# rakhimovv/lvt

Measured on AMD Instinct MI355X. Metric: video-clips/sec/node (VQVAE+DSFVT train step, BAIR 64x64x16), higher is better.
Workload: dtype f32

## Files before the change

### lvt_amd/csrc/attention_flash.hip

```cpp
#include "attn_common.h"

namespace {

template <int I> struct IC { static constexpr int value = I; };
template <int N, int I = 0, class F> __device__ __forceinline__ void static_for(F &&f) {
    if constexpr (I < N) { f(IC<I>{}); static_for<N, I + 1>(f); }
}

typedef _Float16 f16x8 __attribute__((ext_vector_type(8)));
typedef _Float16 f16x2v __attribute__((ext_vector_type(2)));
typedef float f32x2 __attribute__((ext_vector_type(2)));
typedef float f32x4v __attribute__((ext_vector_type(4)));
typedef short s16x4 __attribute__((ext_vector_type(4)));
typedef __attribute__((address_space(3))) s16x4 lds_s16x4;
typedef unsigned u32x4 __attribute__((ext_vector_type(4)));

#define FA_LD 144
#define FA_PL (64 * FA_LD)
#define FA_SLOT (2 * FA_PL)
#define FA_EMIN 30
#define FA_EMAX 254
#define FA_LOG2E 1.4426950408889634f

typedef unsigned u32x2 __attribute__((ext_vector_type(2)));
// ... 13 lines not shown
    v = fa_dpp_max<0x140>(v);
    return v;
}
__device__ __forceinline__ float fa_kg_max(float v) {
    u32x2 r = __builtin_amdgcn_permlane16_swap(__float_as_uint(v), __float_as_uint(v), false, false);
    v = fmaxf(fa_u2f(r[0]), fa_u2f(r[1]));
    r = __builtin_amdgcn_permlane32_swap(__float_as_uint(v), __float_as_uint(v), false, false);
    return fmaxf(fa_u2f(r[0]), fa_u2f(r[1]));
}
__device__ __forceinline__ float fa_kg_sum(float v) {
    u32x2 r = __builtin_amdgcn_permlane16_swap(__float_as_uint(v), __float_as_uint(v), false, false);
    v = fa_u2f(r[0]) + fa_u2f(r[1]);
    r = __builtin_amdgcn_permlane32_swap(__float_as_uint(v), __float_as_uint(v), false, false);
    return fa_u2f(r[0]) + fa_u2f(r[1]);
}
__device__ __forceinline__ float fa_max4(const f32x4v a) { return fmaxf(fmaxf(a[0], a[1]), fmaxf(a[2], a[3])); }
__device__ __forceinline__ float fa_absmax4(const float4 a) { return fmaxf(fmaxf(fabsf(a.x), fabsf(a.y)), fmaxf(fabsf(a.z), fabsf(a.w))); }

__device__ __forceinline__ float fa_mix_lo(unsigned h, float c) {
    float r;
    asm("v_fma_mix_f32 %0, %1, %2, %3 op_sel:[0,0,0] op_sel_hi:[1,0,0]" : "=v"(r) : "v"(h), "v"(-1.f), "v"(c));
    return r;
}
__device__ __forceinline__ float fa_mix_hi(unsigned h, float c) {
    float r;
    asm("v_fma_mix_f32 %0, %1, %2, %3 op_sel:[1,0,0] op_sel_hi:[1,0,0]" : "=v"(r) : "v"(h), "v"(-1.f), "v"(c));
    return r;
}
__device__ __forceinline__ void fa_split_pair(float a, float b, float s, unsigned &ph, unsigned &pl) {
    const f32x2 t = f32x2{a, b} * s;
    ph = __builtin_bit_cast(unsigned, __builtin_convertvector(t, f16x2v));
    const f32x2 r = {fa_mix_lo(ph, t.x), fa_mix_hi(ph, t.y)};
    pl = __builtin_bit_cast(unsigned, __builtin_convertvector(r, f16x2v));
}
__device__ __forceinline__ void fa_split_pair1(float a, float b, unsigned &ph, unsigned &pl) {
    const f32x2 t = {a, b};
    ph = __builtin_bit_cast(unsigned, __builtin_convertvector(t, f16x2v));
    const f32x2 r = {fa_mix_lo(ph, a), fa_mix_hi(ph, b)};
    pl = __builtin_bit_cast(unsigned, __builtin_convertvector(r, f16x2v));
}
__device__ __forceinline__ void fa_split8(const float (&v)[8], f16x8 &h, f16x8 &l) {
    u32x4 uh, ul;
    unsigned a, b;
    fa_split_pair1(v[0], v[1], a, b); uh[0] = a; ul[0] = b;
    fa_split_pair1(v[2], v[3], a, b); uh[1] = a; ul[1] = b;
    fa_split_pair1(v[4], v[5], a, b); uh[2] = a; ul[2] = b;
    fa_split_pair1(v[6], v[7], a, b); uh[3] = a; ul[3] = b;
    h = __builtin_bit_cast(f16x8, uh);
    l = __builtin_bit_cast(f16x8, ul);
}
__device__ __forceinline__ float fa_score(float acc, float kq, float bias) { return fmaf(acc, kq, bias); }
__device__ __forceinline__ f32x4v fa_mfma(const f16x8 a, const f16x8 b, const f32x4v c) {
    return __builtin_amdgcn_mfma_f32_16x16x32_f16(a, b, c, 0, 0, 0);
}

__device__ __forceinline__ int fa_row_scale(const float4 a, const float4 b) {
    return fa_ebits(fa_row16_max(fmaxf(fa_absmax4(a), fa_absmax4(b))));
}
__device__ __forceinline__ void fa_row_store(const float4 a, const float4 b, int eb, unsigned short *slot, float *rs_inv, int row, int c) {
    const float s = fa_u2f((unsigned)(268 - eb) << 23);
    uint2 h0, l0, h1, l1;
    fa_split_pair(a.x, a.y, s, h0.x, l0.x); fa_split_pair(a.z, a.w, s, h0.y, l0.y);
    fa_split_pair(b.x, b.y, s, h1.x, l1.x); fa_split_pair(b.z, b.w, s, h1.y, l1.y);
    unsigned short *d = slot + row * FA_LD + 4 * c;
    *reinterpret_cast<uint2 *>(d) = h0;
    *reinterpret_cast<uint2 *>(d + 64) = h1;
    *reinterpret_cast<uint2 *>(d + FA_PL) = l0;
    *reinterpret_cast<uint2 *>(d + FA_PL + 64) = l1;
    rs_inv[c == 0 ? row : 64 + c] = fa_u2f((unsigned)(eb - 14) << 23);
}
struct G4 { float4 v[4]; };
__device__ __forceinline__ void fa_load(G4 &g, const float *__restrict__ x, const float *__restrict__ y, long long ld, int tid) {
    const int r = tid >> 4, c = tid & 15;
    const float *px = x + (long long)r * ld + 4 * c, *py = y + (long long)r * ld + 4 * c;
    g.v[0] = *reinterpret_cast<const float4 *>(px);
    g.v[1] = *reinterpret_cast<const float4 *>(px + 64);
    g.v[2] = *reinterpret_cast<const float4 *>(py);
    g.v[3] = *reinterpret_cast<const float4 *>(py + 64);
}
__device__ __forceinline__ void fa_park(const G4 &g, unsigned short *slot, float *rs_inv, int tid) {
    const int r = tid >> 4, c = tid & 15;
#pragma unroll
    for (int half = 0; half < 2; ++half)
        fa_row_store(g.v[2 * half], g.v[2 * half + 1], fa_row_scale(g.v[2 * half], g.v[2 * half + 1]), slot, rs_inv, 32 * half + r, c);
}
struct G8 { float4 v[8]; };
__device__ __forceinline__ void fa_load8(G8 &g, const float *__restrict__ x, const float *__restrict__ y, long long ld, int tid) {
    const int r = tid >> 4, c = tid & 15;
    const float *px = x + (long long)r * ld + 4 * c, *py = y + (long long)r * ld + 4 * c;
    g.v[0] = *reinterpret_cast<const float4 *>(px);
    g.v[1] = *reinterpret_cast<const float4 *>(px + 64);
    g.v[2] = *reinterpret_cast<const float4 *>(px + 16 * ld);
    g.v[3] = *reinterpret_cast<const float4 *>(px + 16 * ld + 64);
    g.v[4] = *reinterpret_cast<const float4 *>(py);
    g.v[5] = *reinterpret_cast<const float4 *>(py + 64);
    g.v[6] = *reinterpret_cast<const float4 *>(py + 16 * ld);
    g.v[7] = *reinterpret_cast<const float4 *>(py + 16 * ld + 64);
}
__device__ __forceinline__ void fa_park8(const G8 &g, unsigned short *slot, float *rs_inv, int tid) {
    const int r = tid >> 4, c = tid & 15;
#pragma unroll
    for (int p = 0; p < 4; ++p)
        fa_row_store(g.v[2 * p], g.v[2 * p + 1], fa_row_scale(g.v[2 * p], g.v[2 * p + 1]), slot, rs_inv, 16 * p + r, c);
}
__device__ __forceinline__ void fa_bfrags_request(const float *__restrict__ row, int kg, float4 (&v)[8]) {
#pragma unroll
    for (int s = 0; s < 4; ++s) {
        v[2 * s] = *reinterpret_cast<const float4 *>(row + 32 * s + 8 * kg);
        v[2 * s + 1] = *reinterpret_cast<const float4 *>(row + 32 * s + 8 * kg + 4);
    }
}
__device__ __forceinline__ void fa_bfrags_split(const float4 (&v)[8], f16x8 (&fr)[4][2], float &inv) {
    float m = 0.f;
#pragma unroll
    for (int e = 0; e < 8; ++e) m = fmaxf(m, fa_absmax4(v[e]));
    m = fa_kg_max(m);
    const int eb = fa_ebits(m);
    const float sc = fa_u2f((unsigned)(268 - eb) << 23);
    inv = fa_u2f((unsigned)(eb - 14) << 23);
#pragma unroll
    for (int s = 0; s < 4; ++s) {
        u32x4 uh, ul;
        unsigned a, b;
        fa_split_pair(v[2 * s].x, v[2 * s].y, sc, a, b); uh[0] = a; ul[0] = b;
        fa_split_pair(v[2 * s].z, v[2 * s].w, sc, a, b); uh[1] = a; ul[1] = b;
        fa_split_pair(v[2 * s + 1].x, v[2 * s + 1].y, sc, a, b); uh[2] = a; ul[2] = b;
        fa_split_pair(v[2 * s + 1].z, v[2 * s + 1].w, sc, a, b); uh[3] = a; ul[3] = b;
        fr[s][0] = __builtin_bit_cast(f16x8, uh);
        fr[s][1] = __builtin_bit_cast(f16x8, ul);
    }
}
__device__ __forceinline__ void fa_load_bfrags(const float *__restrict__ row, int kg, f16x8 (&fr)[4][2], float &inv) {
    float4 v[8];
    fa_bfrags_request(row, kg, v);
    fa_bfrags_split(v, fr, inv);
}
__device__ __forceinline__ f16x8 fa_rowfrag(const unsigned short *slot, int pl, int row, int s, int kg) {
    return *reinterpret_cast<const f16x8 *>(slot + pl * FA_PL + row * FA_LD + 32 * s + 8 * kg);
}
__device__ __forceinline__ f16x8 fa_trfrag(const unsigned short *slot, int pl, int rb, int dtile, int c16, int kg) {
    const unsigned short *p = slot + pl * FA_PL + (rb + 4 * kg + (c16 >> 2)) * FA_LD + 16 * dtile + 4 * (c16 & 3);
    const s16x4 lo = __builtin_amdgcn_ds_read_tr16_b64_v4i16((lds_s16x4 *)(p));
    const s16x4 hi = __builtin_amdgcn_ds_read_tr16_b64_v4i16((lds_s16x4 *)(p + 16 * FA_LD));
    union { struct { s16x4 a, b; } s; f16x8 v; } u;
    u.s.a = lo; u.s.b = hi;
    return u.v;
}

struct FaSmem {
    unsigned short ring[2][FA_SLOT];
    float rs_inv[2][80];
    float dhs[32];
};
template <int NR> struct FaSmemA {
    unsigned short ring[2][FA_SLOT];
    float rs_inv[2][80];
    float dhs[32];
    float red[16];
    float R[128 * 4 * NR];
};
struct FaSmem3 {
    unsigned short ring[3][FA_SLOT];
    float rs_inv[3][80];
    float dhs[32];
};

__device__ __forceinline__ int fa_pair(unsigned x) { return (int)(((x >> 4) << 3) | (x & 7)); }
__device__ __forceinline__ int fa_half(unsigned x) { return (int)((x >> 3) & 1); }
__device__ __forceinline__ int fa_pair4(unsigned x) { return (int)(((x >> 5) << 3) | (x & 7)); }
__device__ __forceinline__ int fa_quarter(unsigned x) { return (int)((x >> 3) & 3); }
__device__ __forceinline__ int fa_opaque(int x) { asm volatile("" : "+s"(x)); return x; }

template <int BH, int BW> struct Geo16 {
    static_assert(BW == 16 || BW == 8, "16-wide tiles: BW is 8 or 16");
    static constexpr int HP = BW == 16 ? BH : BH / 2;
    static __device__ __forceinline__ int hj(int hslot, int kg) { return BW == 16 ? hslot : 2 * hslot + (kg >> 1); }
    static __device__ __forceinline__ int wj(int r, int kg) { return BW == 16 ? 4 * kg + r : 4 * (kg & 1) + r; }
};
template <int BT, int BH, int BW> struct BankIdx {
    static constexpr int NT = 2 * BT - 1, NH = 2 * BH - 1, NW = 2 * BW - 1, NB = NT + NH + NW;
};

struct FaArgs {
    const float *q, *k, *v, *d_o;
    long long ld;
    int H;
    float c1, fill2;
    float inv_temper;
    const float *dt, *dh, *dw;
    float *o, *m, *l;
    float *dq, *dk, *dv, *delta, *scal, *bank_partial;
};

template <int BT, int BH, int BW, int MASKED, int NCH>
__device__ __forceinline__ float fa_fwd_body(const FaArgs &A, FaSmem &sm, int bh_, int qhalf) {
    using GE = Geo16<BH, BW>;
    constexpr int HP = GE::HP;
    static_assert(BT * BH * BW == AT_S, "256 tokens");
    const int tid = threadIdx.x, lane = tid & 63, wave = tid >> 6;
    const int c16 = lane & 15, kg = lane >> 4;
    const int b = bh_ / A.H, h = bh_ % A.H;
    const long long row0 = (long long)b * AT_S;
    const int il = wave * 16 + c16, i = qhalf * 128 + il;
    const float *kbase = A.k + row0 * A.ld + h * AT_D, *vbase = A.v + row0 * A.ld + h * AT_D;
    constexpr int NIT = NCH;

    if (tid < 2 * BH - 1) sm.dhs[tid] = A.dh[h * (2 * BH - 1) + tid] * FA_LOG2E;
    G4 g0, g1;
#define FA_G(t) ((((t) & 1) == 0) ? g0 : g1)
    auto load_item = [&](int t, G4 &gg) { fa_load(gg, kbase + (long long)(32 * t) * A.ld, vbase + (long long)(32 * t) * A.ld, A.ld, tid); };
    load_item(0, g0);
    if (NIT > 1) load_item(1, g1);
    f16x8 qb[4][2];
    float qinv;
    fa_load_bfrags(A.q + (row0 + i) * A.ld + h * AT_D, kg, qb, qinv);
    const int wi = i % BW, hi = (i / BW) % BH, ti = i / (BW * BH);
    float bt_[BT], bw_[4];
#pragma unroll
    for (int x = 0; x < BT; ++x) bt_[x] = A.dt[h * (2 * BT - 1) + ti - x + BT - 1] * FA_LOG2E;
#pragma unroll
    for (int r = 0; r < 4; ++r) bw_[r] = A.dw[h * (2 * BW - 1) + wi - GE::wj(r, kg) + BW - 1] * FA_LOG2E;
    const float *dhl = sm.dhs + (hi + BH - 1 - (BW == 16 ? 0 : (kg >> 1)));
    constexpr int HSTEP = BW == 16 ? 1 : 2;
    const float qc = qinv * A.c1;
    fa_park(g0, sm.ring[0], sm.rs_inv[0], tid);
    __syncthreads();

    f32x4v oacc[AT_D / 16];
#pragma unroll
    for (int d = 0; d < AT_D / 16; ++d) oacc[d] = f32x4v{0.f, 0.f, 0.f, 0.f};
    float m_run = -3.0e38f, lsum = 0.f;
    float vmax_run = fa_u2f((unsigned)(FA_EMIN - 14) << 23);

    static_for<NIT>([&](auto tc) {
        constexpr int t = decltype(tc)::value;
        const unsigned short *cur = sm.ring[t & 1];
        const float *cinv = sm.rs_inv[t & 1];
        if constexpr (t + 2 < NIT) load_item(t + 2, FA_G(t));
        f32x4v st[2] = {f32x4v{0.f, 0.f, 0.f, 0.f}, f32x4v{0.f, 0.f, 0.f, 0.f}};
#pragma unroll
        for (int s = 0; s < 4; ++s) {
            f16x8 a[2][2];
#pragma unroll
            for (int kt = 0; kt < 2; ++kt)
#pragma unroll
                for (int pl = 0; pl < 2; ++pl) a[kt][pl] = fa_rowfrag(cur, pl, 16 * kt + c16, s, kg);
#pragma unroll
            for (int kt = 0; kt < 2; ++kt) st[kt] = fa_mfma(a[kt][1], qb[s][0], st[kt]);
#pragma unroll
            for (int kt = 0; kt < 2; ++kt) st[kt] = fa_mfma(a[kt][0], qb[s][1], st[kt]);
#pragma unroll
            for (int kt = 0; kt < 2; ++kt) st[kt] = fa_mfma(a[kt][0], qb[s][0], st[kt]);
        }
        if constexpr (t + 1 < NIT) fa_park(FA_G(t + 1), sm.ring[(t + 1) & 1], sm.rs_inv[(t + 1) & 1], tid);
        float x[8];
        f32x4v vinv[2];
#pragma unroll
        for (int kt = 0; kt < 2; ++kt) {
            const int T = 2 * t + kt;
            const f32x4v kinv = *reinterpret_cast<const f32x4v *>(cinv + 16 * kt + 4 * kg);
            vinv[kt] = *reinterpret_cast<const f32x4v *>(cinv + 32 + 16 * kt + 4 * kg);
            const float bth = bt_[T / HP] + dhl[-HSTEP * (T % HP)];
#pragma unroll
            for (int r = 0; r < 4; ++r) {
                float v = fa_score(st[kt][r], kinv[r] * qc, bth + bw_[r]);
                if (MASKED && 16 * T + 4 * kg + r > i) v = A.fill2;
                x[4 * kt + r] = v;
            }
        }
        float cmax = fmaxf(fmaxf(fmaxf(x[0], x[1]), fmaxf(x[2], x[3])), fmaxf(fmaxf(x[4], x[5]), fmaxf(x[6], x[7])));
        cmax = fa_kg_max(cmax);
        const float vmax_c = fa_kg_max(fmaxf(fa_max4(vinv[0]), fa_max4(vinv[1])));
        const float m_new = fmaxf(m_run, cmax);
        const float alpha = __builtin_amdgcn_exp2f(m_run - m_new);
        m_run = m_new;
        const float vmax_new = fmaxf(vmax_run, vmax_c);
        const float fo = alpha * (vmax_run * __builtin_amdgcn_rcpf(vmax_new));
        vmax_run = vmax_new;
        const float srun = 32768.f * __builtin_amdgcn_rcpf(vmax_new);
        float psum = 0.f, pw[8];
#pragma unroll
        for (int kt = 0; kt < 2; ++kt)
#pragma unroll
            for (int r = 0; r < 4; ++r) {
                const float p = __builtin_amdgcn_exp2f(x[4 * kt + r] - m_new);
                psum += p;
                pw[4 * kt + r] = p * (vinv[kt][r] * srun);
            }
        lsum = lsum * alpha + psum;
        f16x8 pbh, pbl;
        fa_split8(pw, pbh, pbl);
#pragma unroll
        for (int d = 0; d < AT_D / 16; ++d) oacc[d] *= fo;
#pragma unroll
        for (int dp = 0; dp < AT_D / 32; ++dp) {
            f16x8 a[2][2];
#pragma unroll
            for (int dd = 0; dd < 2; ++dd)
#pragma unroll
                for (int pl = 0; pl < 2; ++pl) a[dd][pl] = fa_trfrag(cur, pl, 32, 2 * dp + dd, c16, kg);
#pragma unroll
            for (int dd = 0; dd < 2; ++dd) oacc[2 * dp + dd] = fa_mfma(a[dd][1], pbh, oacc[2 * dp + dd]);
#pragma unroll
            for (int dd = 0; dd < 2; ++dd) oacc[2 * dp + dd] = fa_mfma(a[dd][0], pbl, oacc[2 * dp + dd]);
#pragma unroll
            for (int dd = 0; dd < 2; ++dd) oacc[2 * dp + dd] = fa_mfma(a[dd][0], pbh, oacc[2 * dp + dd]);
        }
        __syncthreads();
    });
#undef FA_G
    const float linv = 1.f / fa_kg_sum(lsum);
    const float osc = (vmax_run * (1.f / 32768.f)) * linv;
    float am = 0.f;
    {
        float *orow = A.o + (row0 + i) * A.ld + h * AT_D + 4 * kg;
#pragma unroll
        for (int d = 0; d < AT_D / 16; ++d) {
            const f32x4v ov = oacc[d] * osc;
            *reinterpret_cast<f32x4v *>(orow + 16 * d) = ov;
            am = fmaxf(am, fmaxf(fmaxf(fabsf(ov[0]), fabsf(ov[1])), fmaxf(fabsf(ov[2]), fabsf(ov[3]))));
        }
    }
    if (kg == 0) {
        const long long si = ((long long)b * A.H + h) * AT_S + i;
        A.m[si] = m_run;
        A.l[si] = linv;
    }
    return am;
}

template <int BT, int BH, int BW, int MASKED>
__global__ __launch_bounds__(512, 1) void lvt_attn_fwd_flash_kernel(const FaArgs A, float *__restrict__ o_amax) {
    __shared__ __attribute__((aligned(16))) FaSmem sm;
    if (threadIdx.x >= 256) __builtin_amdgcn_s_setprio(1);
    float am;
    if (MASKED) {
        am = fa_fwd_body<BT, BH, BW, MASKED, 8>(A, sm, blockIdx.x, 1);
        __syncthreads();
        am = fmaxf(am, fa_fwd_body<BT, BH, BW, MASKED, 4>(A, sm, fa_opaque(blockIdx.x), 0));
    } else {
        am = fa_fwd_body<BT, BH, BW, MASKED, 8>(A, sm, fa_pair(blockIdx.x), fa_half(blockIdx.x));
    }
    if (o_amax) {
        __syncthreads();
        lvt_block_amax_commit(am, o_amax, reinterpret_cast<float *>(sm.ring[0]));
    }
}

template <int BT, int BH, int BW, int MASKED, int NCH, int ONEP>
__device__ __forceinline__ float fa_bwd_a_body(const FaArgs &A, FaSmemA<BT + Geo16<BH, BW>::HP + 4> &sm, int bh_, int qhalf) {
    using GE = Geo16<BH, BW>;
    using BI = BankIdx<BT, BH, BW>;
    constexpr int HP = GE::HP;
    constexpr int NR = BT + HP + 4;
    static_assert(BT * BH * BW == AT_S, "256 tokens");
    const int tid = threadIdx.x, lane = tid & 63, wave = tid >> 6;
    const int c16 = lane & 15, kg = lane >> 4;
    const int b = bh_ / A.H, h = bh_ % A.H;
    const long long row0 = (long long)b * AT_S;
    const int il = wave * 16 + c16, i = qhalf * 128 + il;
    const float *kbase = A.k + row0 * A.ld + h * AT_D, *vbase = A.v + row0 * A.ld + h * AT_D;
    constexpr int NIT = ONEP ? NCH : 2 * NCH;

    if (tid < 2 * BH - 1) sm.dhs[tid] = A.dh[h * (2 * BH - 1) + tid] * FA_LOG2E;
    float *mine = sm.R + (il * 4 + kg) * NR;
#pragma unroll
    for (int x = 0; x < NR; ++x) mine[x] = 0.f;
    G4 g0;
    auto load_item = [&](int t, G4 &gg) {
        const int c = t < NCH ? t : t - NCH;
        fa_load(gg, kbase + (long long)(32 * c) * A.ld, vbase + (long long)(32 * c) * A.ld, A.ld, tid);
    };
    load_item(0, g0);
    f16x8 qb[4][2], dob[4][2];
    float qinv, doinv;
    float4 qraw[8], doraw[8], oraw[ONEP ? 8 : 1];
    fa_bfrags_request(A.q + (row0 + i) * A.ld + h * AT_D, kg, qraw);
    fa_bfrags_request(A.d_o + (row0 + i) * A.ld + h * AT_D, kg, doraw);
    if constexpr (ONEP) fa_bfrags_request(A.o + (row0 + i) * A.ld + h * AT_D, kg, oraw);
    fa_bfrags_split(qraw, qb, qinv);
    fa_bfrags_split(doraw, dob, doinv);
    float delta_early = 0.f;
    if constexpr (ONEP) {
        float a0 = 0.f, a1 = 0.f;
#pragma unroll
        for (int s_ = 0; s_ < 4; ++s_) {
            const float4 o0 = oraw[2 * s_], o1 = oraw[2 * s_ + 1], d0 = doraw[2 * s_], d1 = doraw[2 * s_ + 1];
            a0 = fmaf(o0.x, d0.x, a0); a0 = fmaf(o0.y, d0.y, a0); a0 = fmaf(o0.z, d0.z, a0); a0 = fmaf(o0.w, d0.w, a0);
            a1 = fmaf(o1.x, d1.x, a1); a1 = fmaf(o1.y, d1.y, a1); a1 = fmaf(o1.z, d1.z, a1); a1 = fmaf(o1.w, d1.w, a1);
        }
        delta_early = fa_kg_sum(a0 + a1);
    }
    const long long si = ((long long)b * A.H + h) * AT_S + i;
    const float m_i = A.m[si], linv = A.l[si];
    const int wi = i % BW, hi = (i / BW) % BH, ti = i / (BW * BH);
    float bt_[BT];
    f32x4v bw4;
#pragma unroll
    for (int x = 0; x < BT; ++x) bt_[x] = A.dt[h * (2 * BT - 1) + ti - x + BT - 1] * FA_LOG2E;
#pragma unroll
    for (int r = 0; r < 4; ++r) bw4[r] = A.dw[h * (2 * BW - 1) + wi - GE::wj(r, kg) + BW - 1] * FA_LOG2E;
    const float *dhl = sm.dhs + (hi + BH - 1 - (BW == 16 ? 0 : (kg >> 1)));
    constexpr int HSTEP = BW == 16 ? 1 : 2;
    const float qc = qinv * A.c1;
    fa_park(g0, sm.ring[0], sm.rs_inv[0], tid);
    load_item(1, g0);
    __syncthreads();

    float delta = 0.f, gmax = 0.f;
    float kmax = fa_u2f((unsigned)(FA_EMIN - 14) << 23);
    float sgf = 0.f, kmr = 0.f, dl = 0.f;
    int ebG = FA_EMIN;
    if constexpr (ONEP) { delta = delta_early; dl = delta * linv; }
    f32x4v qacc[AT_D / 16];
#pragma unroll
    for (int d = 0; d < AT_D / 16; ++d) qacc[d] = f32x4v{0.f, 0.f, 0.f, 0.f};
    constexpr bool CORR = ONEP;
    f32x4v cacc[CORR ? AT_D / 16 : 1];
#pragma unroll
    for (int d = 0; d < (CORR ? AT_D / 16 : 1); ++d) cacc[d] = f32x4v{0.f, 0.f, 0.f, 0.f};
    int ebC = 16;
    float rst[BT], rsw[4];
#pragma unroll
    for (int x = 0; x < BT; ++x) rst[x] = 0.f;
#pragma unroll
    for (int r = 0; r < 4; ++r) rsw[r] = 0.f;

    static_for<NIT>([&](auto tc) {
        constexpr int t = decltype(tc)::value;
        constexpr int c = t < NCH ? t : t - NCH;
        constexpr bool PASS2 = ONEP || t >= NCH;
        const unsigned short *cur = sm.ring[t & 1];
        const float *cinv = sm.rs_inv[t & 1];
        constexpr bool PARK = t + 1 < NIT;
        unsigned short *nslot = sm.ring[(t + 1) & 1];
        float *ninv = sm.rs_inv[(t + 1) & 1];
        if constexpr (!ONEP && t == NCH) {
            delta = fa_kg_sum(delta) * linv;
            gmax = fa_kg_max(gmax);
            kmax = fa_kg_max(kmax);
            const float G = gmax + fabsf(delta);
            ebG = fa_ebits(G);
            sgf = fa_u2f((unsigned)(268 - ebG) << 23);
            kmr = __builtin_amdgcn_rcpf(kmax);
            dl = delta * linv;
            float r0 = doinv, r1 = G * qinv;
#pragma unroll
            for (int dd = 32; dd > 0; dd >>= 1) { r0 = fmaxf(r0, __shfl_xor(r0, dd, 64)); r1 = fmaxf(r1, __shfl_xor(r1, dd, 64)); }
            if (lane == 0) { sm.red[wave] = r0; sm.red[8 + wave] = r1; }
        }
        f32x4v st[2] = {f32x4v{0.f, 0.f, 0.f, 0.f}, f32x4v{0.f, 0.f, 0.f, 0.f}};
        f32x4v dp[2] = {f32x4v{0.f, 0.f, 0.f, 0.f}, f32x4v{0.f, 0.f, 0.f, 0.f}};
        int eb0 = 0, eb1 = 0;
        static_for<4>([&](auto sc_) {
            constexpr int s = decltype(sc_)::value;
            f16x8 a[2][2], av[2][2];
#pragma unroll
            for (int kt = 0; kt < 2; ++kt)
#pragma unroll
                for (int pl = 0; pl < 2; ++pl) {
                    a[kt][pl] = fa_rowfrag(cur, pl, 16 * kt + c16, s, kg);
                    av[kt][pl] = fa_rowfrag(cur, pl, 32 + 16 * kt + c16, s, kg);
                }
#pragma unroll
            for (int kt = 0; kt < 2; ++kt) { st[kt] = fa_mfma(a[kt][1], qb[s][0], st[kt]); dp[kt] = fa_mfma(av[kt][1], dob[s][0], dp[kt]); }
#pragma unroll
            for (int kt = 0; kt < 2; ++kt) { st[kt] = fa_mfma(a[kt][0], qb[s][1], st[kt]); dp[kt] = fa_mfma(av[kt][0], dob[s][1], dp[kt]); }
#pragma unroll
            for (int kt = 0; kt < 2; ++kt) { st[kt] = fa_mfma(a[kt][0], qb[s][0], st[kt]); dp[kt] = fa_mfma(av[kt][0], dob[s][0], dp[kt]); }
            if constexpr (PARK) {
                if constexpr (s == 0) eb0 = fa_row_scale(g0.v[0], g0.v[1]);
                if constexpr (s == 1) fa_row_store(g0.v[0], g0.v[1], eb0, nslot, ninv, tid >> 4, tid & 15);
                if constexpr (s == 2) eb1 = fa_row_scale(g0.v[2], g0.v[3]);
                if constexpr (s == 3) fa_row_store(g0.v[2], g0.v[3], eb1, nslot, ninv, 32 + (tid >> 4), tid & 15);
                __builtin_amdgcn_sched_group_barrier(0x100, 8, 0);
#pragma unroll
                for (int e = 0; e < 12; ++e) {
                    __builtin_amdgcn_sched_group_barrier(0x008, 1, 0);
                    __builtin_amdgcn_sched_group_barrier(0x002, (s & 1) ? 3 : 2, 0);
                }
                __builtin_amdgcn_sched_barrier(0);
            }
        });
        if constexpr (t + 2 < NIT) load_item(t + 2, g0);
        float w[8];
        u32x4 pku = {0u, 0u, 0u, 0u};
        if constexpr (CORR) {
            const f32x4v k0 = *reinterpret_cast<const f32x4v *>(cinv + 4 * kg), k1 = *reinterpret_cast<const f32x4v *>(cinv + 16 + 4 * kg);
            const int ebN = max(ebC, (int)(__float_as_uint(fa_kg_max(fmaxf(fa_max4(k0), fa_max4(k1)))) >> 23));
            if (__builtin_amdgcn_ballot_w64(ebN != ebC) != 0) {
                const float f = fa_exp_field(127 + ebC - ebN);
#pragma unroll
                for (int d = 0; d < AT_D / 16; ++d) cacc[d] = cacc[d] * f;
                ebC = ebN;
            }
        }
        const float scc = CORR ? fa_u2f((unsigned)(268 - ebC) << 23) * linv : 0.f;
#pragma unroll
        for (int kt = 0; kt < 2; ++kt) {
            const int T = 2 * c + kt;
            const f32x4v kinv = *reinterpret_cast<const f32x4v *>(cinv + 16 * kt + 4 * kg);
            const f32x4v vinv = *reinterpret_cast<const f32x4v *>(cinv + 32 + 16 * kt + 4 * kg);
            const float bth = bt_[T / HP] + dhl[-HSTEP * (T % HP)];
            if constexpr (!PASS2) kmax = fmaxf(kmax, fa_max4(kinv));
            const f32x4v qk = kinv * qc, bm = bw4 + bth;
            const f32x4v dv = vinv * (PASS2 ? doinv * linv : doinv), kw = kinv * kmr;
            float gt = 0.f;
            const f32x4v ks = kinv * scc;
            f32x4v pkv = {0.f, 0.f, 0.f, 0.f};
#pragma unroll
            for (int r = 0; r < 4; ++r) {
                float x = fa_score(st[kt][r], qk[r], bm[r]);
                if (MASKED && 16 * T + 4 * kg + r > i) x = A.fill2;
                const float ex = __builtin_amdgcn_exp2f(x - m_i);
                if constexpr (!PASS2) {
                    const float dpv = dp[kt][r] * dv[r];
                    delta = fmaf(ex, dpv, delta);
                    gmax = fmaxf(gmax, fabsf(dpv));
                } else {
                    const float g = ex * fmaf(dp[kt][r], dv[r], -dl);
                    gt += g;
                    rsw[r] += g;
                    if constexpr (ONEP) { w[4 * kt + r] = g * kinv[r]; gmax = fmaxf(gmax, fabsf(g)); if constexpr (CORR) pkv[r] = ex * ks[r]; }
                    else w[4 * kt + r] = (g * sgf) * kw[r];
                }
            }
            if constexpr (PASS2) { rst[T / HP] += gt; mine[BT + T % HP] += gt; }
            if constexpr (CORR) {
                pku[2 * kt] = __builtin_bit_cast(unsigned, __builtin_convertvector(f32x2{pkv[0], pkv[1]}, f16x2v));
                pku[2 * kt + 1] = __builtin_bit_cast(unsigned, __builtin_convertvector(f32x2{pkv[2], pkv[3]}, f16x2v));
            }
        }
        if constexpr (PASS2) {
            if constexpr (ONEP) {
                float tm = 0.f;
#pragma unroll
                for (int e = 0; e < 8; ++e) tm = fmaxf(tm, fabsf(w[e]));
                const int ebN = max(ebG, fa_ebits(fa_kg_max(tm)));
                if (__builtin_amdgcn_ballot_w64(ebN != ebG) != 0) {
                    const float f = fa_exp_field(127 + ebG - ebN);
#pragma unroll
                    for (int d = 0; d < AT_D / 16; ++d) qacc[d] = qacc[d] * f;
                    ebG = ebN;
                }
                const float sct = fa_u2f((unsigned)(268 - ebG) << 23);
#pragma unroll
                for (int e = 0; e < 8; ++e) w[e] *= sct;
            }
            f16x8 wbh, wbl;
            fa_split8(w, wbh, wbl);
            const f16x8 pcb = __builtin_bit_cast(f16x8, pku);
#pragma unroll
            for (int dq_ = 0; dq_ < AT_D / 32; ++dq_) {
                f16x8 a[2][2];
#pragma unroll
                for (int dd = 0; dd < 2; ++dd)
#pragma unroll
                    for (int pl = 0; pl < 2; ++pl) a[dd][pl] = fa_trfrag(cur, pl, 0, 2 * dq_ + dd, c16, kg);
#pragma unroll
                for (int dd = 0; dd < 2; ++dd) qacc[2 * dq_ + dd] = fa_mfma(a[dd][1], wbh, qacc[2 * dq_ + dd]);
#pragma unroll
                for (int dd = 0; dd < 2; ++dd) qacc[2 * dq_ + dd] = fa_mfma(a[dd][0], wbl, qacc[2 * dq_ + dd]);
#pragma unroll
                for (int dd = 0; dd < 2; ++dd) qacc[2 * dq_ + dd] = fa_mfma(a[dd][0], wbh, qacc[2 * dq_ + dd]);
                if constexpr (CORR) {
#pragma unroll
                    for (int dd = 0; dd < 2; ++dd) cacc[2 * dq_ + dd] = fa_mfma(a[dd][0], pcb, cacc[2 * dq_ + dd]);
                }
            }
        }
        __syncthreads();
    });
    if constexpr (ONEP) {
        float r0 = doinv, r1 = fa_kg_max(gmax) * qinv;
#pragma unroll
        for (int dd = 32; dd > 0; dd >>= 1) { r0 = fmaxf(r0, __shfl_xor(r0, dd, 64)); r1 = fmaxf(r1, __shfl_xor(r1, dd, 64)); }
        if (lane == 0) { sm.red[wave] = r0; sm.red[8 + wave] = r1; }
        __syncthreads();
    }
    const float f1 = ONEP ? 1.f : kmax, f2 = fa_exp_field(ebG - 14) * A.inv_temper;
    float epsc = 0.f;
    if constexpr (CORR) {
        const float eps = fa_kg_sum((rsw[0] + rsw[1]) + (rsw[2] + rsw[3]));
        delta += eps;
        epsc = (eps * fa_exp_field(ebC - 14)) * A.inv_temper;
    }
    float am = 0.f;
    {
        float *qrow = A.dq + (row0 + i) * A.ld + h * AT_D + 4 * kg;
#pragma unroll
        for (int d = 0; d < AT_D / 16; ++d) {
            f32x4v ov = (qacc[d] * f1) * f2;
            if constexpr (CORR) ov = ov - cacc[d] * epsc;
            *reinterpret_cast<f32x4v *>(qrow + 16 * d) = ov;
            am = fmaxf(am, fmaxf(fmaxf(fabsf(ov[0]), fabsf(ov[1])), fmaxf(fabsf(ov[2]), fabsf(ov[3]))));
        }
    }
    if (kg == 0) A.delta[si] = delta;
    if (tid == 0) {
        float r0 = sm.red[0], r1 = sm.red[8];
#pragma unroll
        for (int x = 1; x < 8; ++x) { r0 = fmaxf(r0, sm.red[x]); r1 = fmaxf(r1, sm.red[8 + x]); }
        A.scal[(bh_ * 2 + qhalf) * 2] = r0;
        A.scal[(bh_ * 2 + qhalf) * 2 + 1] = r1;
    }
    float *R = sm.R;
    float *R2 = reinterpret_cast<float *>(sm.ring[0]);
#pragma unroll
    for (int x = 0; x < BT; ++x) mine[x] = rst[x];
#pragma unroll
    for (int r = 0; r < 4; ++r) mine[BT + HP + r] = rsw[r];
    __syncthreads();
    {
        const int e = tid & 63, part = tid >> 6;
        if (e < BI::NB) {
            float acc = 0.f;
            for (int q = 16 * part; q < 16 * part + 16; ++q) {
                const int iq = qhalf * 128 + q;
                const int wq = iq % BW, hq = (iq / BW) % BH, tq = iq / (BW * BH);
                const float *r = R + (q * 4) * NR;
                if (e < BI::NT) {
                    const int tj = tq - e + BT - 1;
                    if (tj >= 0 && tj < BT) acc += (r[tj] + r[NR + tj]) + (r[2 * NR + tj] + r[3 * NR + tj]);
                } else if (e < BI::NT + BI::NH) {
                    const int hj = hq - (e - BI::NT) + BH - 1;
                    if (hj >= 0 && hj < BH) {
                        if (BW == 16) acc += (r[BT + hj] + r[NR + BT + hj]) + (r[2 * NR + BT + hj] + r[3 * NR + BT + hj]);
                        else acc += r[(2 * (hj & 1)) * NR + BT + (hj >> 1)] + r[(2 * (hj & 1) + 1) * NR + BT + (hj >> 1)];
                    }
                } else {
                    const int wj = wq - (e - BI::NT - BI::NH) + BW - 1;
                    if (wj >= 0 && wj < BW) {
                        if (BW == 16) acc += r[(wj >> 2) * NR + BT + HP + (wj & 3)];
                        else acc += r[(wj >> 2) * NR + BT + HP + (wj & 3)] + r[((wj >> 2) + 2) * NR + BT + HP + (wj & 3)];
                    }
                }
            }
            R2[part * BI::NB + e] = acc;
        }
    }
    __syncthreads();
    if (tid < BI::NB) {
        float acc = 0.f;
#pragma unroll
        for (int part = 0; part < 8; ++part) acc += R2[part * BI::NB + tid];
        A.bank_partial[((long long)bh_ * 2 + qhalf) * BI::NB + tid] = acc;
    }
    return am;
}

template <int BT, int BH, int BW, int MASKED, int ONEP>
__global__ __launch_bounds__(512, 1) void lvt_attn_bwd_flash_a_kernel(const FaArgs A, float *__restrict__ d_amax) {
    __shared__ __attribute__((aligned(16))) FaSmemA<BT + Geo16<BH, BW>::HP + 4> sm;
    if (threadIdx.x >= 256) __builtin_amdgcn_s_setprio(1);
    float am;
    if (MASKED) {
        am = fa_bwd_a_body<BT, BH, BW, MASKED, 8, ONEP>(A, sm, blockIdx.x, 1);
        __syncthreads();
        am = fmaxf(am, fa_bwd_a_body<BT, BH, BW, MASKED, 4, ONEP>(A, sm, fa_opaque(blockIdx.x), 0));
    } else {
        am = fa_bwd_a_body<BT, BH, BW, MASKED, 8, ONEP>(A, sm, fa_pair(blockIdx.x), fa_half(blockIdx.x));
    }
    if (d_amax) {
        __syncthreads();
        lvt_block_amax_commit(am, d_amax, reinterpret_cast<float *>(sm.ring[0]));
    }
}

struct FaSmemB {
    unsigned short ring[2][FA_SLOT];
    unsigned short vres[2][FA_SLOT];
    float rs_inv[2][80];
    float vinv[2][80];
    float dhs[32];
};

template <int BT, int BH, int BW, int MASKED, int C0, int NCH>
__device__ __forceinline__ float fa_bwd_b_body(const FaArgs &A, FaSmemB &sm, int bh_, int khalf) {
    using GE = Geo16<BH, BW>;
    constexpr int HP = GE::HP;
    const int tid = threadIdx.x, lane = tid & 63, wave = tid >> 6;
    const int c16 = lane & 15, kg = lane >> 4;
    const int b = bh_ / A.H, h = bh_ % A.H;
    const long long row0 = (long long)b * AT_S;
    const int jl = wave * 16 + c16, j = khalf * 128 + jl;
    const float *qbase = A.q + row0 * A.ld + h * AT_D, *dobase = A.d_o + row0 * A.ld + h * AT_D;
    const long long sb = ((long long)b * A.H + h) * AT_S;
    constexpr int NIT = NCH;

    if (tid < 2 * BH - 1) sm.dhs[tid] = A.dh[h * (2 * BH - 1) + tid] * FA_LOG2E;
    G4 g0;
    auto load_item = [&](int t, G4 &gg) {
        fa_load(gg, qbase + (long long)(32 * (C0 + t)) * A.ld, dobase + (long long)(32 * (C0 + t)) * A.ld, A.ld, tid);
    };
    {
        const float *rows = A.v + (row0 + khalf * 128) * A.ld + h * AT_D;
        G4 a, bq;
        fa_load(a, rows, rows + 32 * A.ld, A.ld, tid);
        fa_load(bq, rows + 64 * A.ld, rows + 96 * A.ld, A.ld, tid);
        fa_park(a, sm.vres[0], sm.vinv[0], tid);
        fa_park(bq, sm.vres[1], sm.vinv[1], tid);
    }
    f16x8 kb[4][2];
    float kinv;
    load_item(0, g0);
    fa_load_bfrags(A.k + (row0 + j) * A.ld + h * AT_D, kg, kb, kinv);
    const float *sc = A.scal + (long long)bh_ * 4;
    const float domax = fmaxf(sc[0], sc[2]), umax = fmaxf(sc[1], sc[3]);
    const float srun = 32768.f * __builtin_amdgcn_rcpf(domax);
    const int zb = fa_ebits(umax);
    const float zrun = fa_u2f((unsigned)(268 - zb) << 23);
    const unsigned short *vs = sm.vres[jl >> 6];
    const int wj = j % BW, hj = (j / BW) % BH, tj = j / (BW * BH);
    float bt_[BT];
    f32x4v bw4;
#pragma unroll
    for (int x = 0; x < BT; ++x) bt_[x] = A.dt[h * (2 * BT - 1) + x - tj + BT - 1] * FA_LOG2E;
#pragma unroll
    for (int r = 0; r < 4; ++r) bw4[r] = A.dw[h * (2 * BW - 1) + GE::wj(r, kg) - wj + BW - 1] * FA_LOG2E;
    const float *dhl = sm.dhs + (BH - 1 - hj + (BW == 16 ? 0 : (kg >> 1)));
    constexpr int HSTEP = BW == 16 ? 1 : 2;
    const float kc = kinv * A.c1;
    fa_park(g0, sm.ring[0], sm.rs_inv[0], tid);
    if (NIT > 1) load_item(1, g0);
    __syncthreads();
    const float vinv = sm.vinv[jl >> 6][jl & 63];

    f32x4v accv[AT_D / 16], acck[AT_D / 16];
#pragma unroll
    for (int d = 0; d < AT_D / 16; ++d) { accv[d] = f32x4v{0.f, 0.f, 0.f, 0.f}; acck[d] = f32x4v{0.f, 0.f, 0.f, 0.f}; }

    static_for<NIT>([&](auto tc) {
        constexpr int t = decltype(tc)::value;
        constexpr int c = C0 + t;
        constexpr bool PARK = t + 1 < NIT;
        const unsigned short *cur = sm.ring[t & 1];
        const float *cinv = sm.rs_inv[t & 1];
        unsigned short *nslot = sm.ring[(t + 1) & 1];
        float *ninv = sm.rs_inv[(t + 1) & 1];
        f32x4v m4[2], l4[2], d4[2];
#pragma unroll
        for (int qt = 0; qt < 2; ++qt) {
            const long long o = sb + 32 * c + 16 * qt + 4 * kg;
            m4[qt] = *reinterpret_cast<const f32x4v *>(A.m + o);
            l4[qt] = *reinterpret_cast<const f32x4v *>(A.l + o);
            d4[qt] = *reinterpret_cast<const f32x4v *>(A.delta + o);
        }
        f32x4v st[2] = {f32x4v{0.f, 0.f, 0.f, 0.f}, f32x4v{0.f, 0.f, 0.f, 0.f}};
        f32x4v dp[2] = {f32x4v{0.f, 0.f, 0.f, 0.f}, f32x4v{0.f, 0.f, 0.f, 0.f}};
        int eb0 = 0, eb1 = 0;
        f16x8 aq[2][2][2], ad[2][2], vb[2];
        auto load_s = [&](int s_, int bf) {
#pragma unroll
            for (int qt = 0; qt < 2; ++qt)
#pragma unroll
                for (int pl = 0; pl < 2; ++pl) aq[bf][qt][pl] = fa_rowfrag(cur, pl, 16 * qt + c16, s_, kg);
        };
        auto load_p = [&](int s_) {
#pragma unroll
            for (int pl = 0; pl < 2; ++pl) vb[pl] = fa_rowfrag(vs, pl, jl & 63, s_, kg);
#pragma unroll
            for (int qt = 0; qt < 2; ++qt)
#pragma unroll
                for (int pl = 0; pl < 2; ++pl) ad[qt][pl] = fa_rowfrag(cur, pl, 32 + 16 * qt + c16, s_, kg);
        };
        load_s(0, 0);
        static_for<4>([&](auto sc_) {
            constexpr int s = decltype(sc_)::value, bf = s & 1;
            load_p(s);
#pragma unroll
            for (int qt = 0; qt < 2; ++qt) st[qt] = fa_mfma(aq[bf][qt][1], kb[s][0], st[qt]);
#pragma unroll
            for (int qt = 0; qt < 2; ++qt) st[qt] = fa_mfma(aq[bf][qt][0], kb[s][1], st[qt]);
#pragma unroll
            for (int qt = 0; qt < 2; ++qt) st[qt] = fa_mfma(aq[bf][qt][0], kb[s][0], st[qt]);
            if constexpr (s < 3) load_s(s + 1, bf ^ 1);
#pragma unroll
            for (int qt = 0; qt < 2; ++qt) dp[qt] = fa_mfma(ad[qt][1], vb[0], dp[qt]);
#pragma unroll
            for (int qt = 0; qt < 2; ++qt) dp[qt] = fa_mfma(ad[qt][0], vb[1], dp[qt]);
#pragma unroll
            for (int qt = 0; qt < 2; ++qt) dp[qt] = fa_mfma(ad[qt][0], vb[0], dp[qt]);
            if constexpr (PARK) {
                if constexpr (s == 0) eb0 = fa_row_scale(g0.v[0], g0.v[1]);
                if constexpr (s == 1) fa_row_store(g0.v[0], g0.v[1], eb0, nslot, ninv, tid >> 4, tid & 15);
                if constexpr (s == 2) eb1 = fa_row_scale(g0.v[2], g0.v[3]);
                if constexpr (s == 3) fa_row_store(g0.v[2], g0.v[3], eb1, nslot, ninv, 32 + (tid >> 4), tid & 15);
            }
            __builtin_amdgcn_sched_group_barrier(0x100, 6, 0);
#pragma unroll
            for (int e = 0; e < 6; ++e) {
                __builtin_amdgcn_sched_group_barrier(0x008, 1, 0);
                if (PARK) __builtin_amdgcn_sched_group_barrier(0x002, (s & 1) ? 3 : 2, 0);
            }
            if constexpr (s < 3) __builtin_amdgcn_sched_group_barrier(0x100, 4, 0);
#pragma unroll
            for (int e = 0; e < 6; ++e) {
                __builtin_amdgcn_sched_group_barrier(0x008, 1, 0);
                if (PARK) __builtin_amdgcn_sched_group_barrier(0x002, (s & 1) ? 3 : 2, 0);
            }
            __builtin_amdgcn_sched_barrier(0);
        });
        if constexpr (t + 2 < NIT) load_item(t + 2, g0);
        float pw[8], u[8];
#pragma unroll
        for (int qt = 0; qt < 2; ++qt) {
// ... 183 lines not shown
```

Before: 1381.

## Park Q fragments and bias tables in LDS to cut register pressure in bwd-a

The backward-A flash attention kernel now stores the split Q fp16 fragments in a new shared-memory region and reloads them per chunk instead of keeping them in registers. The temporal bias vector moves from a per-thread register array to a shared table. Height-class gradient sums go to a dedicated shared array, reduced across lanes for 16-wide tiles, while the class-sum scratch reuses the Q region after the loop. Opaque and pin asm hints limit rematerialisation and live ranges. The aim is fewer VGPRs and less spilling, at the cost of extra LDS traffic and a larger shared footprint.

```diff
diff --git a/lvt_amd/csrc/attention_flash.hip b/lvt_amd/csrc/attention_flash.hip
--- a/lvt_amd/csrc/attention_flash.hip
+++ b/lvt_amd/csrc/attention_flash.hip
@@ -189,12 +189,15 @@
     float rs_inv[2][80];
     float dhs[32];
 };
-template <int NR> struct FaSmemA {
+#define FA_QPL (128 * FA_LD)
+template <int HT> struct FaSmemA {
     unsigned short ring[2][FA_SLOT];
+    unsigned short qres[2 * FA_QPL];
     float rs_inv[2][80];
     float dhs[32];
+    float dts[16];
     float red[16];
-    float R[128 * 4 * NR];
+    float hs[128 * HT];
 };
 struct FaSmem3 {
     unsigned short ring[3][FA_SLOT];
@@ -207,10 +210,13 @@
 __device__ __forceinline__ int fa_pair4(unsigned x) { return (int)(((x >> 5) << 3) | (x & 7)); }
 __device__ __forceinline__ int fa_quarter(unsigned x) { return (int)((x >> 3) & 3); }
 __device__ __forceinline__ int fa_opaque(int x) { asm volatile("" : "+s"(x)); return x; }
+__device__ __forceinline__ void fa_pin(float &x) { asm volatile("" : "+v"(x)); }
+__device__ __forceinline__ int fa_vopaque(int x) { asm volatile("" : "+v"(x)); return x; }
 
 template <int BH, int BW> struct Geo16 {
     static_assert(BW == 16 || BW == 8, "16-wide tiles: BW is 8 or 16");
     static constexpr int HP = BW == 16 ? BH : BH / 2;
+    static constexpr int HT = BW == 16 ? HP : 4 * HP;
     static __device__ __forceinline__ int hj(int hslot, int kg) { return BW == 16 ? hslot : 2 * hslot + (kg >> 1); }
     static __device__ __forceinline__ int wj(int r, int kg) { return BW == 16 ? 4 * kg + r : 4 * (kg & 1) + r; }
 };
@@ -385,13 +391,14 @@
 }
 
 template <int BT, int BH, int BW, int MASKED, int NCH, int ONEP>
-__device__ __forceinline__ float fa_bwd_a_body(const FaArgs &A, FaSmemA<BT + Geo16<BH, BW>::HP + 4> &sm, int bh_, int qhalf) {
+__device__ __forceinline__ float fa_bwd_a_body(const FaArgs &A, FaSmemA<Geo16<BH, BW>::HT> &sm, int bh_, int qhalf) {
     using GE = Geo16<BH, BW>;
     using BI = BankIdx<BT, BH, BW>;
-    constexpr int HP = GE::HP;
-    constexpr int NR = BT + HP + 4;
+    constexpr int HP = GE::HP, HT = GE::HT;
+    constexpr int NR = BT + 4;
     static_assert(BT * BH * BW == AT_S, "256 tokens");
-    const int tid = threadIdx.x, lane = tid & 63, wave = tid >> 6;
+    static_assert(128 * 4 * NR * 4 <= 2 * FA_QPL * 2, "the class sums R fit in the Q planes");
+    const int tid = fa_vopaque((int)threadIdx.x), lane = tid & 63, wave = tid >> 6;
     const int c16 = lane & 15, kg = lane >> 4;
     const int b = bh_ / A.H, h = bh_ % A.H;
     const long long row0 = (long long)b * AT_S;
@@ -400,9 +407,10 @@
     constexpr int NIT = ONEP ? NCH : 2 * NCH;
 
     if (tid < 2 * BH - 1) sm.dhs[tid] = A.dh[h * (2 * BH - 1) + tid] * FA_LOG2E;
-    float *mine = sm.R + (il * 4 + kg) * NR;
-#pragma unroll
-    for (int x = 0; x < NR; ++x) mine[x] = 0.f;
+    if (tid < 2 * BT - 1) sm.dts[tid] = A.dt[h * (2 * BT - 1) + tid] * FA_LOG2E;
+#pragma unroll
+    for (int x = 0; x < HT / 4; ++x) sm.hs[x * 512 + tid] = 0.f;
+    float *hsl = sm.hs + (BW == 16 ? il * HP : (il * 4 + kg) * HP);
     G4 g0;
     auto load_item = [&](int t, G4 &gg) {
         const int c = t < NCH ? t : t - NCH;
@@ -416,6 +424,10 @@
     fa_bfrags_request(A.d_o + (row0 + i) * A.ld + h * AT_D, kg, doraw);
     if constexpr (ONEP) fa_bfrags_request(A.o + (row0 + i) * A.ld + h * AT_D, kg, oraw);
     fa_bfrags_split(qraw, qb, qinv);
+#pragma unroll
+    for (int s_ = 0; s_ < 4; ++s_)
+#pragma unroll
+        for (int pl = 0; pl < 2; ++pl) *reinterpret_cast<f16x8 *>(sm.qres + pl * FA_QPL + il * FA_LD + 32 * s_ + 8 * kg) = qb[s_][pl];
     fa_bfrags_split(doraw, dob, doinv);
     float delta_early = 0.f;
     if constexpr (ONEP) {
@@ -431,13 +443,11 @@
     const long long si = ((long long)b * A.H + h) * AT_S + i;
     const float m_i = A.m[si], linv = A.l[si];
     const int wi = i % BW, hi = (i / BW) % BH, ti = i / (BW * BH);
-    float bt_[BT];
     f32x4v bw4;
-#pragma unroll
-    for (int x = 0; x < BT; ++x) bt_[x] = A.dt[h * (2 * BT - 1) + ti - x + BT - 1] * FA_LOG2E;
 #pragma unroll
     for (int r = 0; r < 4; ++r) bw4[r] = A.dw[h * (2 * BW - 1) + wi - GE::wj(r, kg) + BW - 1] * FA_LOG2E;
     const float *dhl = sm.dhs + (hi + BH - 1 - (BW == 16 ? 0 : (kg >> 1)));
+    const float *dtl = sm.dts + (ti + BT - 1);
     constexpr int HSTEP = BW == 16 ? 1 : 2;
     const float qc = qinv * A.c1;
     fa_park(g0, sm.ring[0], sm.rs_inv[0], tid);
@@ -491,7 +501,7 @@
         int eb0 = 0, eb1 = 0;
         static_for<4>([&](auto sc_) {
             constexpr int s = decltype(sc_)::value;
-            f16x8 a[2][2], av[2][2];
+            f16x8 a[2][2], av[2][2], qf[2];
 #pragma unroll
             for (int kt = 0; kt < 2; ++kt)
 #pragma unroll
@@ -500,17 +510,19 @@
                     av[kt][pl] = fa_rowfrag(cur, pl, 32 + 16 * kt + c16, s, kg);
                 }
 #pragma unroll
-            for (int kt = 0; kt < 2; ++kt) { st[kt] = fa_mfma(a[kt][1], qb[s][0], st[kt]); dp[kt] = fa_mfma(av[kt][1], dob[s][0], dp[kt]); }
-#pragma unroll
-            for (int kt = 0; kt < 2; ++kt) { st[kt] = fa_mfma(a[kt][0], qb[s][1], st[kt]); dp[kt] = fa_mfma(av[kt][0], dob[s][1], dp[kt]); }
-#pragma unroll
-            for (int kt = 0; kt < 2; ++kt) { st[kt] = fa_mfma(a[kt][0], qb[s][0], st[kt]); dp[kt] = fa_mfma(av[kt][0], dob[s][0], dp[kt]); }
+            for (int pl = 0; pl < 2; ++pl) qf[pl] = *reinterpret_cast<const f16x8 *>(sm.qres + pl * FA_QPL + il * FA_LD + 32 * s + 8 * kg);
+#pragma unroll
+            for (int kt = 0; kt < 2; ++kt) { st[kt] = fa_mfma(a[kt][1], qf[0], st[kt]); dp[kt] = fa_mfma(av[kt][1], dob[s][0], dp[kt]); }
+#pragma unroll
+            for (int kt = 0; kt < 2; ++kt) { st[kt] = fa_mfma(a[kt][0], qf[1], st[kt]); dp[kt] = fa_mfma(av[kt][0], dob[s][1], dp[kt]); }
+#pragma unroll
+            for (int kt = 0; kt < 2; ++kt) { st[kt] = fa_mfma(a[kt][0], qf[0], st[kt]); dp[kt] = fa_mfma(av[kt][0], dob[s][0], dp[kt]); }
             if constexpr (PARK) {
                 if constexpr (s == 0) eb0 = fa_row_scale(g0.v[0], g0.v[1]);
                 if constexpr (s == 1) fa_row_store(g0.v[0], g0.v[1], eb0, nslot, ninv, tid >> 4, tid & 15);
                 if constexpr (s == 2) eb1 = fa_row_scale(g0.v[2], g0.v[3]);
                 if constexpr (s == 3) fa_row_store(g0.v[2], g0.v[3], eb1, nslot, ninv, 32 + (tid >> 4), tid & 15);
-                __builtin_amdgcn_sched_group_barrier(0x100, 8, 0);
+                __builtin_amdgcn_sched_group_barrier(0x100, 10, 0);
 #pragma unroll
                 for (int e = 0; e < 12; ++e) {
                     __builtin_amdgcn_sched_group_barrier(0x008, 1, 0);
@@ -538,7 +550,7 @@
             const int T = 2 * c + kt;
             const f32x4v kinv = *reinterpret_cast<const f32x4v *>(cinv + 16 * kt + 4 * kg);
             const f32x4v vinv = *reinterpret_cast<const f32x4v *>(cinv + 32 + 16 * kt + 4 * kg);
-            const float bth = bt_[T / HP] + dhl[-HSTEP * (T % HP)];
+            const float bth = dtl[-(T / HP)] + dhl[-HSTEP * (T % HP)];
             if constexpr (!PASS2) kmax = fmaxf(kmax, fa_max4(kinv));
             const f32x4v qk = kinv * qc, bm = bw4 + bth;
             const f32x4v dv = vinv * (PASS2 ? doinv * linv : doinv), kw = kinv * kmr;
@@ -562,7 +574,15 @@
                     else w[4 * kt + r] = (g * sgf) * kw[r];
                 }
             }
-            if constexpr (PASS2) { rst[T / HP] += gt; mine[BT + T % HP] += gt; }
+            if constexpr (PASS2) {
+                rst[T / HP] += gt;
+                if constexpr (BW == 16) {
+                    const float gs = fa_kg_sum(gt);
+                    if (kg == 0) hsl[T % HP] += gs;
+                } else {
+                    hsl[T % HP] += gt;
+                }
+            }
             if constexpr (CORR) {
                 pku[2 * kt] = __builtin_bit_cast(unsigned, __builtin_convertvector(f32x2{pkv[0], pkv[1]}, f16x2v));
                 pku[2 * kt + 1] = __builtin_bit_cast(unsigned, __builtin_convertvector(f32x2{pkv[2], pkv[3]}, f16x2v));
@@ -606,8 +626,18 @@
                 }
             }
         }
+#pragma unroll
+        for (int x = 0; x < BT; ++x) fa_pin(rst[x]);
+#pragma unroll
+        for (int r = 0; r < 4; ++r) fa_pin(rsw[r]);
+        fa_pin(gmax);
+        if constexpr (!PASS2) { fa_pin(delta); fa_pin(kmax); }
         __syncthreads();
     });
+    {
+    const int tid_ = fa_vopaque(tid), lane = tid_ & 63, wave = tid_ >> 6, kg = lane >> 4;
+    const int il = wave * 16 + (lane & 15), i = qhalf * 128 + il;
+    const long long si = ((long long)b * A.H + h) * AT_S + i;
     if constexpr (ONEP) {
         float r0 = doinv, r1 = fa_kg_max(gmax) * qinv;
 #pragma unroll
@@ -634,22 +664,23 @@
         }
     }
     if (kg == 0) A.delta[si] = delta;
-    if (tid == 0) {
+    if (tid_ == 0) {
         float r0 = sm.red[0], r1 = sm.red[8];
 #pragma unroll
         for (int x = 1; x < 8; ++x) { r0 = fmaxf(r0, sm.red[x]); r1 = fmaxf(r1, sm.red[8 + x]); }
         A.scal[(bh_ * 2 + qhalf) * 2] = r0;
         A.scal[(bh_ * 2 + qhalf) * 2 + 1] = r1;
     }
-    float *R = sm.R;
+    float *R = reinterpret_cast<float *>(sm.qres);
     float *R2 = reinterpret_cast<float *>(sm.ring[0]);
+    float *mine = R + (il * 4 + kg) * NR;
 #pragma unroll
     for (int x = 0; x < BT; ++x) mine[x] = rst[x];
 #pragma unroll
-    for (int r = 0; r < 4; ++r) mine[BT + HP + r] = rsw[r];
+    for (int r = 0; r < 4; ++r) mine[BT + r] = rsw[r];
     __syncthreads();
     {
-        const int e = tid & 63, part = tid >> 6;
+        const int e = tid_ & 63, part = tid_ >> 6;
         if (e < BI::NB) {
             float acc = 0.f;
             for (int q = 16 * part; q < 16 * part + 16; ++q) {
@@ -662,14 +693,15 @@
                 } else if (e < BI::NT + BI::NH) {
                     const int hj = hq - (e - BI::NT) + BH - 1;
                     if (hj >= 0 && hj < BH) {
-                        if (BW == 16) acc += (r[BT + hj] + r[NR + BT + hj]) + (r[2 * NR + BT + hj] + r[3 * NR + BT + hj]);
-                        else acc += r[(2 * (hj & 1)) * NR + BT + (hj >> 1)] + r[(2 * (hj & 1) + 1) * NR + BT + (hj >> 1)];
+                        const float *hq_ = sm.hs + q * HT;
+                        if (BW == 16) acc += hq_[hj];
+                        else acc += hq_[(2 * (hj & 1)) * HP + (hj >> 1)] + hq_[(2 * (hj & 1) + 1) * HP + (hj >> 1)];
                     }
                 } else {
                     const int wj = wq - (e - BI::NT - BI::NH) + BW - 1;
                     if (wj >= 0 && wj < BW) {
-                        if (BW == 16) acc += r[(wj >> 2) * NR + BT + HP + (wj & 3)];
-                        else acc += r[(wj >> 2) * NR + BT + HP + (wj & 3)] + r[((wj >> 2) + 2) * NR + BT + HP + (wj & 3)];
+                        if (BW == 16) acc += r[(wj >> 2) * NR + BT + (wj & 3)];
+                        else acc += r[(wj >> 2) * NR + BT + (wj & 3)] + r[((wj >> 2) + 2) * NR + BT + (wj & 3)];
                     }
                 }
             }
@@ -677,18 +709,20 @@
         }
     }
     __syncthreads();
-    if (tid < BI::NB) {
+    if (tid_ < BI::NB) {
         float acc = 0.f;
 #pragma unroll
-        for (int part = 0; part < 8; ++part) acc += R2[part * BI::NB + tid];
-        A.bank_partial[((long long)bh_ * 2 + qhalf) * BI::NB + tid] = acc;
-    }
+        for (int part = 0; part < 8; ++part) acc += R2[part * BI::NB + tid_];
+        A.bank_partial[((long long)bh_ * 2 + qhalf) * BI::NB + tid_] = acc;
+    }
+    fa_pin(am);
     return am;
+    }
 }
 
 template <int BT, int BH, int BW, int MASKED, int ONEP>
 __global__ __launch_bounds__(512, 1) void lvt_attn_bwd_flash_a_kernel(const FaArgs A, float *__restrict__ d_amax) {
-    __shared__ __attribute__((aligned(16))) FaSmemA<BT + Geo16<BH, BW>::HP + 4> sm;
+    __shared__ __attribute__((aligned(16))) FaSmemA<Geo16<BH, BW>::HT> sm;
     if (threadIdx.x >= 256) __builtin_amdgcn_s_setprio(1);
     float am;
     if (MASKED) {
```

Result: no change. 1394 (median of 6 runs) (+0.9%).
